# stanfordnlp/mac-network

Measured on NVIDIA H100. Metric: mac_reasoning_steps_per_sec, higher is better.
Workload: dtype bf16

## Files before the change

### mac_network_b200/csrc/read_step.cuh

```cuda
#pragma once
#include "tc_gemm.cuh"

namespace mac {

constexpr int RS_D = 512;
constexpr int RS_BM = 64;
constexpr int RS_KB = RS_D / TC_BK;
constexpr int RS_BLK = RS_BM * TC_BK * 2;
constexpr int RS_A_BYTES = RS_KB * RS_BLK;
constexpr int RS_B_HALF = 256 * TC_BK * 2;
constexpr int RS_W_BYTES = 2 * RS_B_HALF;
constexpr int RS_STAGE = RS_W_BYTES + RS_BLK;
constexpr int RS_STAGES = 2;
constexpr int RS_Q_SLOT = RS_KB;
constexpr int RS_SLOTS = RS_Q_SLOT + 1 + RS_KB;
constexpr int RS_CONSUMERS = 256;
constexpr int RS_THREADS = RS_CONSUMERS + 32;
constexpr int RS_SMEM_BYTES = RS_A_BYTES + RS_STAGES * RS_STAGE + 1024  + 64  +
                              2 * RS_BM * 4  + 2 * RS_D * 4  +
                              2 * RS_D * 4 ;
static_assert(RS_SMEM_BYTES <= 232448, "over the sm_90 per-block shared memory opt-in limit");
static_assert(RS_STAGE % 1024 == 0 && RS_W_BYTES % 1024 == 0, "swizzled operands need 1024-byte alignment");

__device__ __forceinline__ float bf16lo(uint32_t w) { return __uint_as_float(w << 16); }
__device__ __forceinline__ float bf16hi(uint32_t w) { return __uint_as_float(w & 0xffff0000u); }

__device__ __forceinline__ void wgmma_bf16_n256(float (&d)[128], uint64_t adesc, uint64_t bdesc, uint32_t accum) {
  asm volatile(
      "{\n\t.reg .pred p;\n\t"
      "setp.ne.b32 p, %130, 0;\n\t"
      "wgmma.mma_async.sync.aligned.m64n256k16.f32.bf16.bf16 "
      "{%0, %1, %2, %3, %4, %5, %6, %7, %8, %9, %10, %11, %12, %13, %14, %15, %16, %17, %18, %19, %20, %21, %22, %23, %24, %25, %26, %27, %28, %29, %30, %31, %32, %33, %34, %35, %36, %37, %38, %39, %40, %41, %42, %43, %44, %45, %46, %47, %48, %49, %50, %51, %52, %53, %54, %55, %56, %57, %58, %59, %60, %61, %62, %63, %64, %65, %66, %67, %68, %69, %70, %71, %72, %73, %74, %75, %76, %77, %78, %79, %80, %81, %82, %83, %84, %85, %86, %87, %88, %89, %90, %91, %92, %93, %94, %95, %96, %97, %98, %99, %100, %101, %102, %103, %104, %105, %106, %107, %108, %109, %110, %111, %112, %113, %114, %115, %116, %117, %118, %119, %120, %121, %122, %123, %124, %125, %126, %127}, %128, %129, p, 1, 1, 0, 0;\n\t}"
      : "+f"(d[0]), "+f"(d[1]), "+f"(d[2]), "+f"(d[3]), "+f"(d[4]), "+f"(d[5]), "+f"(d[6]), "+f"(d[7]), "+f"(d[8]), "+f"(d[9]), "+f"(d[10]), "+f"(d[11]), "+f"(d[12]), "+f"(d[13]), "+f"(d[14]), "+f"(d[15]), "+f"(d[16]), "+f"(d[17]), "+f"(d[18]), "+f"(d[19]), "+f"(d[20]), "+f"(d[21]), "+f"(d[22]), "+f"(d[23]), "+f"(d[24]), "+f"(d[25]), "+f"(d[26]), "+f"(d[27]), "+f"(d[28]), "+f"(d[29]), "+f"(d[30]), "+f"(d[31]), "+f"(d[32]), "+f"(d[33]), "+f"(d[34]), "+f"(d[35]), "+f"(d[36]), "+f"(d[37]), "+f"(d[38]), "+f"(d[39]), "+f"(d[40]), "+f"(d[41]), "+f"(d[42]), "+f"(d[43]), "+f"(d[44]), "+f"(d[45]), "+f"(d[46]), "+f"(d[47]), "+f"(d[48]), "+f"(d[49]), "+f"(d[50]), "+f"(d[51]), "+f"(d[52]), "+f"(d[53]), "+f"(d[54]), "+f"(d[55]), "+f"(d[56]), "+f"(d[57]), "+f"(d[58]), "+f"(d[59]), "+f"(d[60]), "+f"(d[61]), "+f"(d[62]), "+f"(d[63]), "+f"(d[64]), "+f"(d[65]), "+f"(d[66]), "+f"(d[67]), "+f"(d[68]), "+f"(d[69]), "+f"(d[70]), "+f"(d[71]), "+f"(d[72]), "+f"(d[73]), "+f"(d[74]), "+f"(d[75]), "+f"(d[76]), "+f"(d[77]), "+f"(d[78]), "+f"(d[79]), "+f"(d[80]), "+f"(d[81]), "+f"(d[82]), "+f"(d[83]), "+f"(d[84]), "+f"(d[85]), "+f"(d[86]), "+f"(d[87]), "+f"(d[88]), "+f"(d[89]), "+f"(d[90]), "+f"(d[91]), "+f"(d[92]), "+f"(d[93]), "+f"(d[94]), "+f"(d[95]), "+f"(d[96]), "+f"(d[97]), "+f"(d[98]), "+f"(d[99]), "+f"(d[100]), "+f"(d[101]), "+f"(d[102]), "+f"(d[103]), "+f"(d[104]), "+f"(d[105]), "+f"(d[106]), "+f"(d[107]), "+f"(d[108]), "+f"(d[109]), "+f"(d[110]), "+f"(d[111]), "+f"(d[112]), "+f"(d[113]), "+f"(d[114]), "+f"(d[115]), "+f"(d[116]), "+f"(d[117]), "+f"(d[118]), "+f"(d[119]), "+f"(d[120]), "+f"(d[121]), "+f"(d[122]), "+f"(d[123]), "+f"(d[124]), "+f"(d[125]), "+f"(d[126]), "+f"(d[127])
      : "l"(adesc), "l"(bdesc), "r"(accum));
}
inline bool read_step_supported(int B, int N, int d) {
  return d == RS_D && N >= 1 && N <= 256 && B >= 1 && B < (1 << 22);
}

struct ReadStepParams {
  int M, N;
  const float* y;
  const float* ctrl;
  const float* bm2;
  const float* wr;
  float* logits;
};

__device__ __forceinline__ void rs_consumer_bar() { asm volatile("bar.sync 1, %0;" ::"n"(RS_CONSUMERS) : "memory"); }

__global__ void __launch_bounds__(RS_THREADS, 1)
read_step_kernel(const __grid_constant__ CUtensorMap map_p, const __grid_constant__ CUtensorMap map_q,
                 const __grid_constant__ CUtensorMap map_w1, const __grid_constant__ CUtensorMap map_w2,
                 const ReadStepParams p) {
  extern __shared__ unsigned char smem_dyn[];
  const uint32_t base_u32 = smem_u32(smem_dyn);
  unsigned char* a_tile = smem_dyn + ((1024u - (base_u32 & 1023u)) & 1023u);
  unsigned char* b_ring = a_tile + RS_A_BYTES;
  uint64_t* full = reinterpret_cast<uint64_t*>(b_ring + RS_STAGES * RS_STAGE);
  uint64_t* empty = full + RS_STAGES;
  float* s_lg = reinterpret_cast<float*>(full + 8);
  float* s_ctrl = s_lg + 2 * RS_BM;
  float* s_bm2 = s_ctrl + 2 * RS_D;
  float* s_wr = s_bm2 + RS_D;

  const int warp = threadIdx.x >> 5, lane = threadIdx.x & 31;
  const int row0 = blockIdx.x * RS_BM;
  const int s_lo = row0 / p.N;

  if (threadIdx.x == RS_CONSUMERS) {
    tma_prefetch_desc(&map_p);
    tma_prefetch_desc(&map_q);
    tma_prefetch_desc(&map_w1);
    tma_prefetch_desc(&map_w2);
    for (int i = 0; i < RS_STAGES; ++i) {
      mbar_init(&full[i], 1);
      mbar_init(&empty[i], RS_CONSUMERS / 32);
    }
    fence_mbar_init();
  }
  __syncthreads();

  if (warp == RS_CONSUMERS / 32) {
    if (elect_one()) {
      for (int j = 0; j < RS_SLOTS; ++j) {
        const int s = j % RS_STAGES;
        mbar_wait(&empty[s], ((j / RS_STAGES) & 1) ^ 1);
        unsigned char* dst = b_ring + s * RS_STAGE;
        if (j == RS_Q_SLOT) {
          mbar_expect_tx(&full[s], RS_A_BYTES);
          for (int kb = 0; kb < RS_KB; ++kb) tma_load_2d(dst + kb * RS_BLK, &map_q, kb * TC_BK, row0, &full[s]);
          continue;
        }
        const bool g1 = j < RS_Q_SLOT;
        mbar_expect_tx(&full[s], g1 ? RS_W_BYTES + RS_BLK : RS_W_BYTES);
        const CUtensorMap* m = g1 ? &map_w1 : &map_w2;
        const int k0 = (g1 ? j : j - RS_Q_SLOT - 1) * TC_BK;
        if (g1) tma_load_2d(dst + RS_W_BYTES, &map_p, k0, row0, &full[s]);
        tma_load_2d(dst, m, k0, 0, &full[s]);
        tma_load_2d(dst + RS_B_HALF, m, k0, 256, &full[s]);
      }
    }
    return;
  }

  const int tid = threadIdx.x;
  const int g = warp >> 2;
  const int rl = 16 * (warp & 3) + (lane >> 2);
  const int cq = 256 * g + 2 * (lane & 3);
  const int prow = tid >> 3;
  const int poff = prow * 128 + (tid & 7) * 16;
  const int pcol = ((tid & 7) ^ (prow & 7)) << 3;
  for (int i = tid; i < RS_D; i += RS_CONSUMERS) {
    s_bm2[i] = __ldg(p.bm2 + i);
    s_wr[i] = __ldg(p.wr + i);
  }
  float acc[128];
  const int last_row = min(p.M, row0 + RS_BM) - 1;
  const int nsamp = last_row / p.N - s_lo + 1;
  for (int q = 0; q < min(nsamp, 2); ++q)
    for (int i = tid; i < RS_D; i += RS_CONSUMERS) s_ctrl[q * RS_D + i] = __ldg(p.ctrl + (size_t)(s_lo + q) * RS_D + i);
  int yoff[2];
#pragma unroll
  for (int u = 0; u < 2; ++u) yoff[u] = min(row0 + prow + 32 * u, p.M - 1) / p.N * RS_D + pcol;

  for (int j = 0; j < RS_KB; ++j) {
    const int s = j % RS_STAGES;
    unsigned char* stage = b_ring + s * RS_STAGE;
    float4 y0[2], y1[2];
#pragma unroll
    for (int u = 0; u < 2; ++u) {
      y0[u] = *reinterpret_cast<const float4*>(p.y + yoff[u] + j * TC_BK);
      y1[u] = *reinterpret_cast<const float4*>(p.y + yoff[u] + j * TC_BK + 4);
    }
    mbar_wait(&full[s], (j / RS_STAGES) & 1);
#pragma unroll
    for (int u = 0; u < 2; ++u) {
      uint4* c = reinterpret_cast<uint4*>(stage + RS_W_BYTES + poff + u * 32 * 128);
      const uint4 v = *c;
      *c = make_uint4(pack_bf16(bf16lo(v.x) * y0[u].x, bf16hi(v.x) * y0[u].y), pack_bf16(bf16lo(v.y) * y0[u].z, bf16hi(v.y) * y0[u].w),
                      pack_bf16(bf16lo(v.z) * y1[u].x, bf16hi(v.z) * y1[u].y), pack_bf16(bf16lo(v.w) * y1[u].z, bf16hi(v.w) * y1[u].w));
    }
    fence_proxy_async();
    rs_consumer_bar();
    const uint64_t adesc = make_sw128_kmajor_desc(smem_u32(stage + RS_W_BYTES));
    const uint64_t bdesc = make_sw128_kmajor_desc(smem_u32(stage + g * RS_B_HALF));
    wgmma_fence();
#pragma unroll
    for (int k = 0; k < TC_BK / 16; ++k) wgmma_bf16_n256(acc, adesc + 2 * k, bdesc + 2 * k, (j || k) ? 1u : 0u);
    wgmma_commit();
    wgmma_wait<1>();
    wgmma_hold(acc);
    if (j && lane == 0) mbar_arrive(&empty[(j - 1) % RS_STAGES]);
  }
  wgmma_wait<0>();
  wgmma_hold(acc);
  if (lane == 0) mbar_arrive(&empty[(RS_KB - 1) % RS_STAGES]);

  constexpr int qs = RS_Q_SLOT % RS_STAGES;
  const unsigned char* q_tile = b_ring + qs * RS_STAGE;
  mbar_wait(&full[qs], (RS_Q_SLOT / RS_STAGES) & 1);
#pragma unroll
  for (int h = 0; h < 2; ++h) {
    const int r = rl + 8 * h, row = row0 + r;
#pragma unroll
    for (int j = 0; j < 32; ++j) {
      const int n = cq + 8 * j;
      const int kb = n >> 6, c = (n & 63) >> 3;
      const int off = kb * RS_BLK + r * 128 + ((c ^ (r & 7)) << 4) + (n & 7) * 2;
      const uint32_t q = *reinterpret_cast<const uint32_t*>(q_tile + off);
      const uint32_t hv = row < p.M ? pack_bf16(elu_fast(acc[4 * j + 2 * h] + bf16lo(q)), elu_fast(acc[4 * j + 2 * h + 1] + bf16hi(q)))
                                    : 0u;
      *reinterpret_cast<uint32_t*>(a_tile + off) = hv;
    }
  }
  fence_proxy_async();
  rs_consumer_bar();
  if (lane == 0) mbar_arrive(&empty[qs]);

  const uint32_t a_u = smem_u32(a_tile);
  for (int j = 0; j < RS_KB; ++j) {
    const int jj = RS_Q_SLOT + 1 + j, s = jj % RS_STAGES;
    mbar_wait(&full[s], (jj / RS_STAGES) & 1);
    const uint64_t adesc = make_sw128_kmajor_desc(a_u + j * RS_BLK);
    const uint64_t bdesc = make_sw128_kmajor_desc(smem_u32(b_ring + s * RS_STAGE + g * RS_B_HALF));
    wgmma_fence();
#pragma unroll
    for (int k = 0; k < TC_BK / 16; ++k) wgmma_bf16_n256(acc, adesc + 2 * k, bdesc + 2 * k, (j || k) ? 1u : 0u);
    wgmma_commit();
    wgmma_wait<1>();
    wgmma_hold(acc);
    if (j && lane == 0) mbar_arrive(&empty[(jj - 1) % RS_STAGES]);
  }
  wgmma_wait<0>();
  wgmma_hold(acc);
  if (lane == 0) mbar_arrive(&empty[(RS_SLOTS - 1) % RS_STAGES]);

#pragma unroll
  for (int h = 0; h < 2; ++h) {
    const int r = rl + 8 * h, row = row0 + r;
    const int s = min(row, p.M - 1) / p.N;
    const float* crow = s - s_lo < 2 ? s_ctrl + (s - s_lo) * RS_D : p.ctrl + (size_t)s * RS_D;
    float part = 0.f;
#pragma unroll
    for (int j = 0; j < 32; ++j) {
      const int n = cq + 8 * j;
      const float2 cc = *reinterpret_cast<const float2*>(crow + n);
      const float2 bb = *reinterpret_cast<const float2*>(s_bm2 + n);
      const float2 ww = *reinterpret_cast<const float2*>(s_wr + n);
      const float t0 = elu_fast((acc[4 * j + 2 * h] + bb.x) * cc.x);
      const float t1 = elu_fast((acc[4 * j + 2 * h + 1] + bb.y) * cc.y);
      part = fmaf(t0, ww.x, part);
      part = fmaf(t1, ww.y, part);
    }
    part += __shfl_xor_sync(0xffffffffu, part, 1);
    part += __shfl_xor_sync(0xffffffffu, part, 2);
    if ((lane & 3) == 0) s_lg[g * RS_BM + r] = part;
  }
  rs_consumer_bar();
  if (tid < RS_BM && row0 + tid < p.M) p.logits[row0 + tid] = s_lg[tid] + s_lg[RS_BM + tid];
}

inline int read_step_launch(const void* inv, const void* kb_bf16, const float* y, const float* control,
                            const mac_read_weights* w, float* att, float* info, int B, int N, int d, cudaStream_t stream) {
  if (!read_step_supported(B, N, d)) return MAC_ERR_UNSUPPORTED;
  if (!inv || !kb_bf16 || !y || !control || !w->Wm_bf16 || !w->Wm2_bf16 || !att || !info) return MAC_ERR_INVALID;
  const int M = B * N;
  const TcReadScratch s = tc_read_scratch(const_cast<void*>(inv), B, N, d);
  CUtensorMap mp, mq, mw1, mw2;
  int st = make_tmap_2d(&mp, s.P, 1, (uint64_t)M, (uint64_t)d, (uint64_t)d * 2, RS_BM, TC_BK, 1);
  if (st != MAC_OK) return st;
  st = make_tmap_2d(&mq, s.Q, 1, (uint64_t)M, (uint64_t)d, (uint64_t)d * 2, RS_BM, TC_BK, 1);
  if (st != MAC_OK) return st;
  st = make_tmap_2d(&mw1, w->Wm_bf16, 1, (uint64_t)d, (uint64_t)d, (uint64_t)2 * d * 2, 256, TC_BK, 1);
  if (st != MAC_OK) return st;
  st = make_tmap_2d(&mw2, w->Wm2_bf16, 1, (uint64_t)d, (uint64_t)d, (uint64_t)d * 2, 256, TC_BK, 1);
  if (st != MAC_OK) return st;
  ReadStepParams p{};
  p.M = M; p.N = N; p.y = y; p.ctrl = control; p.bm2 = w->bm2; p.wr = w->wr; p.logits = s.parts;
  MAC_CUDA_TRY(cudaFuncSetAttribute(read_step_kernel, cudaFuncAttributeMaxDynamicSharedMemorySize, RS_SMEM_BYTES));
  read_step_kernel<<<(M + RS_BM - 1) / RS_BM, RS_THREADS, RS_SMEM_BYTES, stream>>>(mp, mq, mw1, mw2, p);
  MAC_LAUNCH_CHECK();
  return mac_kb_attend_fwd(s.parts, 1, w->br, kb_bf16, 1, att, info, B, N, d, stream);
}

}
```

### mac_network_b200/csrc/read_step_fp8.cuh

```cuda
#pragma once
#include <cuda_fp8.h>
#include <cuda_fp16.h>
#include "read_step.cuh"

namespace mac {

constexpr int R8_BK = 128;
constexpr int R8_KB = RS_D / R8_BK;
constexpr int R8_BLK = RS_BM * R8_BK;
constexpr int R8_A_BYTES = R8_KB * R8_BLK;
constexpr int R8_B_HALF = 256 * R8_BK;
constexpr int R8_W_BYTES = 2 * R8_B_HALF;
constexpr int R8_STAGE = R8_W_BYTES + R8_BLK;
constexpr int R8_STAGES = 2;
constexpr int R8_Q_SLOT = R8_KB;
constexpr int R8_SLOTS = R8_Q_SLOT + 1 + R8_KB;
constexpr int R8_SMEM_BYTES = R8_A_BYTES + R8_STAGES * R8_STAGE + 1024  + 64  +
                              2 * RS_BM * 4  + 2 * RS_BM * 4  +
                              2 * RS_D * 4  + 2 * RS_D * 4  +
                              4 * RS_D * 4  + 2 * RS_BM * 4 ;
static_assert(RS_A_BYTES <= R8_STAGE, "the bf16 Q tile must fit in one ring stage");
static_assert(R8_SMEM_BYTES <= 232448, "over the sm_90 per-block shared memory opt-in limit");
static_assert(R8_STAGE % 1024 == 0 && R8_A_BYTES % 1024 == 0, "swizzled operands need 1024-byte alignment");

__device__ __forceinline__ void wgmma_e4m3_n256(float (&d)[128], uint64_t adesc, uint64_t bdesc, uint32_t accum) {
  asm volatile(
      "{\n\t.reg .pred p;\n\t"
      "setp.ne.b32 p, %130, 0;\n\t"
      "wgmma.mma_async.sync.aligned.m64n256k32.f32.e4m3.e4m3 "
      "{%0, %1, %2, %3, %4, %5, %6, %7, %8, %9, %10, %11, %12, %13, %14, %15, %16, %17, %18, %19, %20, %21, %22, %23, %24, %25, %26, %27, %28, %29, %30, %31, %32, %33, %34, %35, %36, %37, %38, %39, %40, %41, %42, %43, %44, %45, %46, %47, %48, %49, %50, %51, %52, %53, %54, %55, %56, %57, %58, %59, %60, %61, %62, %63, %64, %65, %66, %67, %68, %69, %70, %71, %72, %73, %74, %75, %76, %77, %78, %79, %80, %81, %82, %83, %84, %85, %86, %87, %88, %89, %90, %91, %92, %93, %94, %95, %96, %97, %98, %99, %100, %101, %102, %103, %104, %105, %106, %107, %108, %109, %110, %111, %112, %113, %114, %115, %116, %117, %118, %119, %120, %121, %122, %123, %124, %125, %126, %127}, %128, %129, p, 1, 1;\n\t}"
      : "+f"(d[0]), "+f"(d[1]), "+f"(d[2]), "+f"(d[3]), "+f"(d[4]), "+f"(d[5]), "+f"(d[6]), "+f"(d[7]), "+f"(d[8]), "+f"(d[9]), "+f"(d[10]), "+f"(d[11]), "+f"(d[12]), "+f"(d[13]), "+f"(d[14]), "+f"(d[15]), "+f"(d[16]), "+f"(d[17]), "+f"(d[18]), "+f"(d[19]), "+f"(d[20]), "+f"(d[21]), "+f"(d[22]), "+f"(d[23]), "+f"(d[24]), "+f"(d[25]), "+f"(d[26]), "+f"(d[27]), "+f"(d[28]), "+f"(d[29]), "+f"(d[30]), "+f"(d[31]), "+f"(d[32]), "+f"(d[33]), "+f"(d[34]), "+f"(d[35]), "+f"(d[36]), "+f"(d[37]), "+f"(d[38]), "+f"(d[39]), "+f"(d[40]), "+f"(d[41]), "+f"(d[42]), "+f"(d[43]), "+f"(d[44]), "+f"(d[45]), "+f"(d[46]), "+f"(d[47]), "+f"(d[48]), "+f"(d[49]), "+f"(d[50]), "+f"(d[51]), "+f"(d[52]), "+f"(d[53]), "+f"(d[54]), "+f"(d[55]), "+f"(d[56]), "+f"(d[57]), "+f"(d[58]), "+f"(d[59]), "+f"(d[60]), "+f"(d[61]), "+f"(d[62]), "+f"(d[63]), "+f"(d[64]), "+f"(d[65]), "+f"(d[66]), "+f"(d[67]), "+f"(d[68]), "+f"(d[69]), "+f"(d[70]), "+f"(d[71]), "+f"(d[72]), "+f"(d[73]), "+f"(d[74]), "+f"(d[75]), "+f"(d[76]), "+f"(d[77]), "+f"(d[78]), "+f"(d[79]), "+f"(d[80]), "+f"(d[81]), "+f"(d[82]), "+f"(d[83]), "+f"(d[84]), "+f"(d[85]), "+f"(d[86]), "+f"(d[87]), "+f"(d[88]), "+f"(d[89]), "+f"(d[90]), "+f"(d[91]), "+f"(d[92]), "+f"(d[93]), "+f"(d[94]), "+f"(d[95]), "+f"(d[96]), "+f"(d[97]), "+f"(d[98]), "+f"(d[99]), "+f"(d[100]), "+f"(d[101]), "+f"(d[102]), "+f"(d[103]), "+f"(d[104]), "+f"(d[105]), "+f"(d[106]), "+f"(d[107]), "+f"(d[108]), "+f"(d[109]), "+f"(d[110]), "+f"(d[111]), "+f"(d[112]), "+f"(d[113]), "+f"(d[114]), "+f"(d[115]), "+f"(d[116]), "+f"(d[117]), "+f"(d[118]), "+f"(d[119]), "+f"(d[120]), "+f"(d[121]), "+f"(d[122]), "+f"(d[123]), "+f"(d[124]), "+f"(d[125]), "+f"(d[126]), "+f"(d[127])
      : "l"(adesc), "l"(bdesc), "r"(accum));
}

__device__ __forceinline__ float2 e4m3x2_to_float2(uint32_t v) {
  const __half2_raw h = __nv_cvt_fp8x2_to_halfraw2((__nv_fp8x2_storage_t)(v & 0xffffu), __NV_E4M3);
  return __half22float2(*reinterpret_cast<const __half2*>(&h));
}
__device__ __forceinline__ uint32_t float2_to_e4m3x2(float a, float b) {
  return (uint32_t)__nv_cvt_float2_to_fp8x2(make_float2(a, b), __NV_SATFINITE, __NV_E4M3);
}
__device__ __forceinline__ uint32_t scale4_e4m3(uint32_t w, float4 y, float sc) {
  const float2 a = e4m3x2_to_float2(w), b = e4m3x2_to_float2(w >> 16);
  return float2_to_e4m3x2(a.x * (y.x * sc), a.y * (y.y * sc)) | (float2_to_e4m3x2(b.x * (y.z * sc), b.y * (y.w * sc)) << 16);
}

struct ReadStepFp8Params {
  int M, N;
  const float* y;
  const float* ctrl;
  const float* bm2;
  const float* wr;
  const float* sP;
  const float* sw1;
  const float* sw2;
  float* logits;
};

__global__ void __launch_bounds__(RS_THREADS, 1)
read_step_fp8_kernel(const __grid_constant__ CUtensorMap map_p8, const __grid_constant__ CUtensorMap map_q,
                     const __grid_constant__ CUtensorMap map_w1, const __grid_constant__ CUtensorMap map_w2,
                     const ReadStepFp8Params p) {
  extern __shared__ unsigned char smem_dyn[];
  const uint32_t base_u32 = smem_u32(smem_dyn);
  unsigned char* a_tile = smem_dyn + ((1024u - (base_u32 & 1023u)) & 1023u);
  unsigned char* b_ring = a_tile + R8_A_BYTES;
  uint64_t* full = reinterpret_cast<uint64_t*>(b_ring + R8_STAGES * R8_STAGE);
  uint64_t* empty = full + R8_STAGES;
  float* s_lg = reinterpret_cast<float*>(full + 8);
  float* s_hmax = s_lg + 2 * RS_BM;
  float* s_ctrl = s_hmax + 2 * RS_BM;
  float* s_ys = s_ctrl + 2 * RS_D;
  float* s_bm2 = s_ys + 2 * RS_D;
  float* s_wr = s_bm2 + RS_D;
  float* s_sw1 = s_wr + RS_D;
  float* s_sw2 = s_sw1 + RS_D;
  float* s_ay = s_sw2 + RS_D;
  float* s_iay = s_ay + RS_BM;

  const int warp = threadIdx.x >> 5, lane = threadIdx.x & 31;
  const int row0 = blockIdx.x * RS_BM;
  const int s_lo = row0 / p.N;

  if (threadIdx.x == RS_CONSUMERS) {
    tma_prefetch_desc(&map_p8);
    tma_prefetch_desc(&map_q);
    tma_prefetch_desc(&map_w1);
    tma_prefetch_desc(&map_w2);
    for (int i = 0; i < R8_STAGES; ++i) {
      mbar_init(&full[i], 1);
      mbar_init(&empty[i], RS_CONSUMERS / 32);
    }
    fence_mbar_init();
  }
  __syncthreads();

  if (warp == RS_CONSUMERS / 32) {
    if (elect_one()) {
      for (int j = 0; j < R8_SLOTS; ++j) {
        const int s = j % R8_STAGES;
        mbar_wait(&empty[s], ((j / R8_STAGES) & 1) ^ 1);
        unsigned char* dst = b_ring + s * R8_STAGE;
        if (j == R8_Q_SLOT) {
          mbar_expect_tx(&full[s], RS_A_BYTES);
          for (int kb = 0; kb < RS_KB; ++kb) tma_load_2d(dst + kb * RS_BLK, &map_q, kb * TC_BK, row0, &full[s]);
          continue;
        }
        const bool g1 = j < R8_Q_SLOT;
        mbar_expect_tx(&full[s], g1 ? R8_W_BYTES + R8_BLK : R8_W_BYTES);
        const CUtensorMap* m = g1 ? &map_w1 : &map_w2;
        const int k0 = (g1 ? j : j - R8_Q_SLOT - 1) * R8_BK;
        if (g1) tma_load_2d(dst + R8_W_BYTES, &map_p8, k0, row0, &full[s]);
        tma_load_2d(dst, m, k0, 0, &full[s]);
        tma_load_2d(dst + R8_B_HALF, m, k0, 256, &full[s]);
      }
    }
    return;
  }

  const int tid = threadIdx.x;
  const int g = warp >> 2;
  const int rl = 16 * (warp & 3) + (lane >> 2);
  const int cq = 256 * g + 2 * (lane & 3);
  const int prow = tid >> 3;
  const int poff = prow * 128 + (tid & 7) * 16;
  const int pcol = ((tid & 7) ^ (prow & 7)) << 4;
  for (int i = tid; i < RS_D; i += RS_CONSUMERS) {
    s_bm2[i] = __ldg(p.bm2 + i);
    s_wr[i] = __ldg(p.wr + i);
    s_sw1[i] = __ldg(p.sw1 + i);
    s_sw2[i] = __ldg(p.sw2 + i);
  }
  const int last_row = min(p.M, row0 + RS_BM) - 1;
  const int nsamp = last_row / p.N - s_lo + 1;
  for (int q = 0; q < min(nsamp, 2); ++q)
    for (int i = tid; i < RS_D; i += RS_CONSUMERS) s_ctrl[q * RS_D + i] = __ldg(p.ctrl + (size_t)(s_lo + q) * RS_D + i);
  for (int q = warp; q < nsamp; q += RS_CONSUMERS / 32) {
    const float* yr = p.y + (size_t)(s_lo + q) * RS_D;
    float v[RS_D / 32];
    float m = 0.f;
#pragma unroll
    for (int i = 0; i < RS_D / 32; ++i) {
      v[i] = __ldg(yr + lane + 32 * i);
      m = fmaxf(m, fabsf(v[i]));
    }
    m = warp_max(m);
    const float inv = m > 0.f ? 1.f / m : 0.f;
    if (lane == 0) {
      s_ay[q] = m;
      s_iay[q] = inv;
    }
    if (q < 2) {
#pragma unroll
      for (int i = 0; i < RS_D / 32; ++i) s_ys[q * RS_D + lane + 32 * i] = v[i] * inv;
    }
  }
  rs_consumer_bar();
  const float* yrow[2];
  float ysc[2];
#pragma unroll
  for (int u = 0; u < 2; ++u) {
    const int q = min(row0 + prow + 32 * u, p.M - 1) / p.N - s_lo;
    yrow[u] = (q < 2 ? s_ys + q * RS_D : p.y + (size_t)(s_lo + q) * RS_D) + pcol;
    ysc[u] = q < 2 ? 1.f : s_iay[q];
  }

  float acc[128];
  for (int j = 0; j < R8_KB; ++j) {
    const int s = j % R8_STAGES;
    unsigned char* stage = b_ring + s * R8_STAGE;
    mbar_wait(&full[s], (j / R8_STAGES) & 1);
#pragma unroll
    for (int u = 0; u < 2; ++u) {
      uint4* c = reinterpret_cast<uint4*>(stage + R8_W_BYTES + poff + u * 32 * 128);
      const uint4 v = *c;
      const float* yr = yrow[u] + j * R8_BK;
      const float4 y0 = *reinterpret_cast<const float4*>(yr), y1 = *reinterpret_cast<const float4*>(yr + 4);
      const float4 y2 = *reinterpret_cast<const float4*>(yr + 8), y3 = *reinterpret_cast<const float4*>(yr + 12);
      *c = make_uint4(scale4_e4m3(v.x, y0, ysc[u]), scale4_e4m3(v.y, y1, ysc[u]), scale4_e4m3(v.z, y2, ysc[u]),
                      scale4_e4m3(v.w, y3, ysc[u]));
    }
    fence_proxy_async();
    rs_consumer_bar();
    const uint64_t adesc = make_sw128_kmajor_desc(smem_u32(stage + R8_W_BYTES));
    const uint64_t bdesc = make_sw128_kmajor_desc(smem_u32(stage + g * R8_B_HALF));
    wgmma_fence();
#pragma unroll
    for (int k = 0; k < R8_BK / 32; ++k) wgmma_e4m3_n256(acc, adesc + 2 * k, bdesc + 2 * k, (j || k) ? 1u : 0u);
    wgmma_commit();
    wgmma_wait<1>();
    wgmma_hold(acc);
    if (j && lane == 0) mbar_arrive(&empty[(j - 1) % R8_STAGES]);
  }
  wgmma_wait<0>();
  wgmma_hold(acc);
  if (lane == 0) mbar_arrive(&empty[(R8_KB - 1) % R8_STAGES]);

  constexpr int qs = R8_Q_SLOT % R8_STAGES;
  const unsigned char* q_tile = b_ring + qs * R8_STAGE;
  mbar_wait(&full[qs], (R8_Q_SLOT / R8_STAGES) & 1);
#pragma unroll
  for (int h = 0; h < 2; ++h) {
    const int r = rl + 8 * h, row = row0 + r;
    const int rr = min(row, p.M - 1);
    const float rf = __ldg(p.sP + rr) * s_ay[rr / p.N - s_lo];
    float m = 0.f;
#pragma unroll
    for (int j = 0; j < 32; ++j) {
      const int n = cq + 8 * j;
      const int kb = n >> 6, c = (n & 63) >> 3;
      const uint32_t q = *reinterpret_cast<const uint32_t*>(q_tile + kb * RS_BLK + r * 128 + ((c ^ (r & 7)) << 4) + (n & 7) * 2);
      const float2 sw = *reinterpret_cast<const float2*>(s_sw1 + n);
      float h0 = elu_fast(acc[4 * j + 2 * h] * rf * sw.x + bf16lo(q));
      float h1 = elu_fast(acc[4 * j + 2 * h + 1] * rf * sw.y + bf16hi(q));
      if (row >= p.M) h0 = h1 = 0.f;
      acc[4 * j + 2 * h] = h0;
      acc[4 * j + 2 * h + 1] = h1;
      m = fmaxf(m, fmaxf(fabsf(h0), fabsf(h1)));
    }
    m = fmaxf(m, __shfl_xor_sync(0xffffffffu, m, 1));
    m = fmaxf(m, __shfl_xor_sync(0xffffffffu, m, 2));
    if ((lane & 3) == 0) s_hmax[g * RS_BM + r] = m;
  }
  rs_consumer_bar();
  if (lane == 0) mbar_arrive(&empty[qs]);
#pragma unroll
  for (int h = 0; h < 2; ++h) {
    const int r = rl + 8 * h;
    const float am = fmaxf(s_hmax[r], s_hmax[RS_BM + r]);
    const float inv = am > 0.f ? 448.f / am : 0.f;
#pragma unroll
    for (int j = 0; j < 32; ++j) {
      const int n = cq + 8 * j;
      const int kb = n >> 7, c = (n & 127) >> 4;
      *reinterpret_cast<uint16_t*>(a_tile + kb * R8_BLK + r * 128 + ((c ^ (r & 7)) << 4) + (n & 15)) =
          (uint16_t)float2_to_e4m3x2(acc[4 * j + 2 * h] * inv, acc[4 * j + 2 * h + 1] * inv);
    }
  }
  fence_proxy_async();
  rs_consumer_bar();

  const uint32_t a_u = smem_u32(a_tile);
  for (int j = 0; j < R8_KB; ++j) {
    const int jj = R8_Q_SLOT + 1 + j, s = jj % R8_STAGES;
    mbar_wait(&full[s], (jj / R8_STAGES) & 1);
    const uint64_t adesc = make_sw128_kmajor_desc(a_u + j * R8_BLK);
    const uint64_t bdesc = make_sw128_kmajor_desc(smem_u32(b_ring + s * R8_STAGE + g * R8_B_HALF));
    wgmma_fence();
#pragma unroll
    for (int k = 0; k < R8_BK / 32; ++k) wgmma_e4m3_n256(acc, adesc + 2 * k, bdesc + 2 * k, (j || k) ? 1u : 0u);
    wgmma_commit();
    wgmma_wait<1>();
    wgmma_hold(acc);
    if (j && lane == 0) mbar_arrive(&empty[(jj - 1) % R8_STAGES]);
  }
  wgmma_wait<0>();
  wgmma_hold(acc);
  if (lane == 0) mbar_arrive(&empty[(R8_SLOTS - 1) % R8_STAGES]);

#pragma unroll
  for (int h = 0; h < 2; ++h) {
    const int r = rl + 8 * h, row = row0 + r;
    const int s = min(row, p.M - 1) / p.N;
    const float* crow = s - s_lo < 2 ? s_ctrl + (s - s_lo) * RS_D : p.ctrl + (size_t)s * RS_D;
    const float sh = fmaxf(s_hmax[r], s_hmax[RS_BM + r]) / 448.f;
    float part = 0.f;
#pragma unroll
    for (int j = 0; j < 32; ++j) {
      const int n = cq + 8 * j;
      const float2 cc = *reinterpret_cast<const float2*>(crow + n);
      const float2 bb = *reinterpret_cast<const float2*>(s_bm2 + n);
      const float2 ww = *reinterpret_cast<const float2*>(s_wr + n);
      const float2 sw = *reinterpret_cast<const float2*>(s_sw2 + n);
      const float t0 = elu_fast((acc[4 * j + 2 * h] * sh * sw.x + bb.x) * cc.x);
      const float t1 = elu_fast((acc[4 * j + 2 * h + 1] * sh * sw.y + bb.y) * cc.y);
      part = fmaf(t0, ww.x, part);
      part = fmaf(t1, ww.y, part);
    }
    part += __shfl_xor_sync(0xffffffffu, part, 1);
    part += __shfl_xor_sync(0xffffffffu, part, 2);
    if ((lane & 3) == 0) s_lg[g * RS_BM + r] = part;
  }
  rs_consumer_bar();
  if (tid < RS_BM && row0 + tid < p.M) p.logits[row0 + tid] = s_lg[tid] + s_lg[RS_BM + tid];
}

__global__ void pack_weight_fp8_kernel(const float* __restrict__ W, uint8_t* __restrict__ Wt, float* __restrict__ col_scale,
                                       int K, int N) {
  __shared__ float tile[32][33];
  __shared__ float s_max[8][32];
  const int n0 = blockIdx.x * 32, tx = threadIdx.x, ty = threadIdx.y;
  float m = 0.f;
  if (n0 + tx < N)
    for (int k = ty; k < K; k += 8) m = fmaxf(m, fabsf(W[(size_t)k * N + n0 + tx]));
  s_max[ty][tx] = m;
  __syncthreads();
  if (ty == 0) {
    for (int i = 1; i < 8; ++i) m = fmaxf(m, s_max[i][tx]);
    s_max[0][tx] = m;
    if (n0 + tx < N) col_scale[n0 + tx] = m / 448.f;
  }
  __syncthreads();
  for (int k0 = 0; k0 < K; k0 += 32) {
    for (int i = ty; i < 32; i += 8) {
      const int k = k0 + i, n = n0 + tx;
      tile[i][tx] = (k < K && n < N) ? W[(size_t)k * N + n] : 0.f;
    }
    __syncthreads();
    for (int i = ty; i < 32; i += 8) {
      const int n = n0 + i, k = k0 + tx;
      const float am = s_max[0][i];
      if (n < N && k < K)
        Wt[(size_t)n * K + k] = am > 0.f ? __nv_cvt_float_to_fp8(tile[tx][i] / (am / 448.f), __NV_SATFINITE, __NV_E4M3) : 0;
    }
    __syncthreads();
  }
}

__global__ void __launch_bounds__(256) quant_rows_e4m3_kernel(const __nv_bfloat16* __restrict__ P, uint8_t* __restrict__ P8,
                                                             float* __restrict__ sP, int M) {
  const int m = blockIdx.x * 8 + (threadIdx.x >> 5), lane = threadIdx.x & 31;
  if (m >= M) return;
  const uint4* src = reinterpret_cast<const uint4*>(P + (size_t)m * RS_D) + 2 * lane;
  const uint4 a = src[0], b = src[1];
  const uint32_t w[8] = {a.x, a.y, a.z, a.w, b.x, b.y, b.z, b.w};
  float v[16];
  float am = 0.f;
#pragma unroll
  for (int i = 0; i < 8; ++i) {
    v[2 * i] = bf16lo(w[i]);
    v[2 * i + 1] = bf16hi(w[i]);
    am = fmaxf(am, fmaxf(fabsf(v[2 * i]), fabsf(v[2 * i + 1])));
  }
  am = warp_max(am);
  const float s = am / 448.f;
  uint32_t o[4];
#pragma unroll
  for (int i = 0; i < 4; ++i) {
    const uint32_t lo = float2_to_e4m3x2(v[4 * i] / s, v[4 * i + 1] / s);
    const uint32_t hi = float2_to_e4m3x2(v[4 * i + 2] / s, v[4 * i + 3] / s);
    o[i] = am > 0.f ? lo | (hi << 16) : 0u;
  }
  reinterpret_cast<uint4*>(P8 + (size_t)m * RS_D)[lane] = make_uint4(o[0], o[1], o[2], o[3]);
  if (lane == 0) sP[m] = s;
}

struct Fp8ReadScratch {
  uint8_t* P8;
  float* sP;
  __nv_bfloat16* Q;
  float* parts;
  __nv_bfloat16* P;
};
inline size_t fp8_align1k(size_t b) { return (b + 1023) & ~(size_t)1023; }
inline size_t fp8_read_invariant_bytes(int B, int N, int d) {
  const size_t M = (size_t)B * N;
  return fp8_align1k(M * d) + fp8_align1k(M * 4) + 2 * fp8_align1k(M * d * 2) + fp8_align1k(M * 4) + 1024;
}
inline Fp8ReadScratch fp8_read_scratch(void* inv, int B, int N, int d) {
  const size_t M = (size_t)B * N;
  char* o = tc_align1k(inv);
  Fp8ReadScratch s;
  s.P8 = reinterpret_cast<uint8_t*>(o);
  o += fp8_align1k(M * d);
  s.sP = reinterpret_cast<float*>(o);
  o += fp8_align1k(M * 4);
  s.Q = reinterpret_cast<__nv_bfloat16*>(o);
  o += fp8_align1k(M * d * 2);
  s.parts = reinterpret_cast<float*>(o);
  o += fp8_align1k(M * 4);
  s.P = reinterpret_cast<__nv_bfloat16*>(o);
  return s;
}

inline int fp8_read_invariant(const void* kb_bf16, const mac_read_weights* w, void* inv, size_t inv_bytes, int B, int N, int d,
                              cudaStream_t stream) {
  if (!read_step_supported(B, N, d)) return MAC_ERR_UNSUPPORTED;
  if (!kb_bf16 || !w->Wx_bf16 || !w->Wm_bf16) return MAC_ERR_INVALID;
  if (inv_bytes < fp8_read_invariant_bytes(B, N, d)) return MAC_ERR_WORKSPACE;
  const int M = B * N;
  const Fp8ReadScratch s = fp8_read_scratch(inv, B, N, d);
  TcGemmParams p{};
  p.M = M; p.N = d; p.rows_per_batch = N; p.ldo = d;
  p.epi = TC_EPI_ACT; p.act = MAC_ACT_NON; p.bias = w->bx; p.out0 = s.P;
  int st = tc_gemm_launch(kb_bf16, d, nullptr, 0, w->Wx_bf16, p, stream);
  if (st != MAC_OK) return st;
  p.bias = w->bm; p.out0 = s.Q;
  st = tc_gemm_launch(s.P, d, nullptr, 0, reinterpret_cast<const __nv_bfloat16*>(w->Wm_bf16) + d, p, stream, nullptr, 2 * d);
  if (st != MAC_OK) return st;
  quant_rows_e4m3_kernel<<<(M + 7) / 8, 256, 0, stream>>>(s.P, s.P8, s.sP, M);
  MAC_LAUNCH_CHECK();
  return MAC_OK;
}

inline int read_step_fp8_launch(const void* inv, const void* kb_bf16, const float* y, const float* control,
                                const mac_read_weights* w, float* att, float* info, int B, int N, int d, cudaStream_t stream) {
  if (!read_step_supported(B, N, d)) return MAC_ERR_UNSUPPORTED;
  if (!inv || !kb_bf16 || !y || !control || !w->Wm_fp8 || !w->Wm_fp8_scale || !w->Wm2_fp8 || !w->Wm2_fp8_scale || !att || !info)
    return MAC_ERR_INVALID;
  const int M = B * N;
  const Fp8ReadScratch s = fp8_read_scratch(const_cast<void*>(inv), B, N, d);
  CUtensorMap mp, mq, mw1, mw2;
  int st = make_tmap_2d(&mp, s.P8, 2, (uint64_t)M, (uint64_t)d, (uint64_t)d, RS_BM, R8_BK, 1);
  if (st != MAC_OK) return st;
  st = make_tmap_2d(&mq, s.Q, 1, (uint64_t)M, (uint64_t)d, (uint64_t)d * 2, RS_BM, TC_BK, 1);
  if (st != MAC_OK) return st;
  st = make_tmap_2d(&mw1, w->Wm_fp8, 2, (uint64_t)d, (uint64_t)d, (uint64_t)d, 256, R8_BK, 1);
  if (st != MAC_OK) return st;
  st = make_tmap_2d(&mw2, w->Wm2_fp8, 2, (uint64_t)d, (uint64_t)d, (uint64_t)d, 256, R8_BK, 1);
  if (st != MAC_OK) return st;
  ReadStepFp8Params p{};
  p.M = M; p.N = N; p.y = y; p.ctrl = control; p.bm2 = w->bm2; p.wr = w->wr;
  p.sP = s.sP; p.sw1 = w->Wm_fp8_scale; p.sw2 = w->Wm2_fp8_scale; p.logits = s.parts;
  MAC_CUDA_TRY(cudaFuncSetAttribute(read_step_fp8_kernel, cudaFuncAttributeMaxDynamicSharedMemorySize, R8_SMEM_BYTES));
  read_step_fp8_kernel<<<(M + RS_BM - 1) / RS_BM, RS_THREADS, R8_SMEM_BYTES, stream>>>(mp, mq, mw1, mw2, p);
  MAC_LAUNCH_CHECK();
  return mac_kb_attend_fwd(s.parts, 1, w->br, kb_bf16, 1, att, info, B, N, d, stream);
}

}
```

Before: 17800.

## Double read-step row tile so each warpgroup owns 64 rows over split N

The bf16 read-step kernel moves from a 64-row tile, where two warpgroups split the 512 output columns, to a 128-row tile where each warpgroup owns 64 rows and walks the two 256-column halves in sequence. Each ring stage now holds one 256-wide weight half, so every weight byte loaded serves twice as many rows. The Q tile goes straight into the A buffer through its own mbarrier. A four-warp producer warpgroup uses setmaxnreg to hand registers to the consumers. The epilogue writes logits directly, without cross-warpgroup shared reductions, and the fp8 kernel gets its own tile constants so it keeps its old geometry. The cost is twice as many ring slots per tile, half as many CTAs (so less parallelism at small M), and heavier register pressure.

New measurement: 18170 (median of 6 runs). 2.1% higher.

```diff
diff --git a/mac_network_b200/csrc/read_step.cuh b/mac_network_b200/csrc/read_step.cuh
--- a/mac_network_b200/csrc/read_step.cuh
+++ b/mac_network_b200/csrc/read_step.cuh
@@ -4,23 +4,26 @@
 namespace mac {
 
 constexpr int RS_D = 512;
-constexpr int RS_BM = 64;
+constexpr int RS_BM = 128;
+constexpr int RS_WG_BM = 64;
 constexpr int RS_KB = RS_D / TC_BK;
 constexpr int RS_BLK = RS_BM * TC_BK * 2;
+constexpr int RS_WG_BLK = RS_WG_BM * TC_BK * 2;
 constexpr int RS_A_BYTES = RS_KB * RS_BLK;
 constexpr int RS_B_HALF = 256 * TC_BK * 2;
-constexpr int RS_W_BYTES = 2 * RS_B_HALF;
-constexpr int RS_STAGE = RS_W_BYTES + RS_BLK;
+constexpr int RS_STAGE = RS_B_HALF + RS_BLK;
 constexpr int RS_STAGES = 2;
-constexpr int RS_Q_SLOT = RS_KB;
-constexpr int RS_SLOTS = RS_Q_SLOT + 1 + RS_KB;
+constexpr int RS_G2_SLOT = 2 * RS_KB;
+constexpr int RS_SLOTS = 4 * RS_KB;
 constexpr int RS_CONSUMERS = 256;
-constexpr int RS_THREADS = RS_CONSUMERS + 32;
-constexpr int RS_SMEM_BYTES = RS_A_BYTES + RS_STAGES * RS_STAGE + 1024  + 64  +
-                              2 * RS_BM * 4  + 2 * RS_D * 4  +
-                              2 * RS_D * 4 ;
+constexpr int RS_THREADS = RS_CONSUMERS + 128;
+constexpr int RS_PRODUCER_REGS = 40;
+constexpr int RS_CONSUMER_REGS = 232;
+constexpr int RS_SMEM_BYTES = RS_A_BYTES + RS_STAGES * RS_STAGE + 1024  + 64 ;
 static_assert(RS_SMEM_BYTES <= 232448, "over the sm_90 per-block shared memory opt-in limit");
-static_assert(RS_STAGE % 1024 == 0 && RS_W_BYTES % 1024 == 0, "swizzled operands need 1024-byte alignment");
+static_assert(4 * RS_D * 4 <= RS_WG_BLK, "epilogue 2's staged operands fill a warpgroup's rows of a P block");
+static_assert(RS_STAGE % 1024 == 0 && RS_BLK % 1024 == 0 && RS_WG_BLK % 1024 == 0,
+              "swizzled operands need 1024-byte alignment");
 
 __device__ __forceinline__ float bf16lo(uint32_t w) { return __uint_as_float(w << 16); }
 __device__ __forceinline__ float bf16hi(uint32_t w) { return __uint_as_float(w & 0xffff0000u); }
@@ -47,7 +50,10 @@
   float* logits;
 };
 
-__device__ __forceinline__ void rs_consumer_bar() { asm volatile("bar.sync 1, %0;" ::"n"(RS_CONSUMERS) : "memory"); }
+__device__ __forceinline__ void rs_warpgroup_bar(int g) {
+  if (g) asm volatile("bar.sync 2, 128;" ::: "memory");
+  else asm volatile("bar.sync 1, 128;" ::: "memory");
+}
 
 __global__ void __launch_bounds__(RS_THREADS, 1)
 read_step_kernel(const __grid_constant__ CUtensorMap map_p, const __grid_constant__ CUtensorMap map_q,
@@ -59,14 +65,10 @@
   unsigned char* b_ring = a_tile + RS_A_BYTES;
   uint64_t* full = reinterpret_cast<uint64_t*>(b_ring + RS_STAGES * RS_STAGE);
   uint64_t* empty = full + RS_STAGES;
-  float* s_lg = reinterpret_cast<float*>(full + 8);
-  float* s_ctrl = s_lg + 2 * RS_BM;
-  float* s_bm2 = s_ctrl + 2 * RS_D;
-  float* s_wr = s_bm2 + RS_D;
+  uint64_t* q_full = empty + RS_STAGES;
 
   const int warp = threadIdx.x >> 5, lane = threadIdx.x & 31;
   const int row0 = blockIdx.x * RS_BM;
-  const int s_lo = row0 / p.N;
 
   if (threadIdx.x == RS_CONSUMERS) {
     tma_prefetch_desc(&map_p);
@@ -77,148 +79,155 @@
       mbar_init(&full[i], 1);
       mbar_init(&empty[i], RS_CONSUMERS / 32);
     }
+    mbar_init(q_full, 1);
     fence_mbar_init();
   }
   __syncthreads();
 
-  if (warp == RS_CONSUMERS / 32) {
-    if (elect_one()) {
+  if (warp >= RS_CONSUMERS / 32) {
+    asm volatile("setmaxnreg.dec.sync.aligned.u32 %0;" ::"n"(RS_PRODUCER_REGS));
+    if (warp == RS_CONSUMERS / 32 && elect_one()) {
       for (int j = 0; j < RS_SLOTS; ++j) {
         const int s = j % RS_STAGES;
         mbar_wait(&empty[s], ((j / RS_STAGES) & 1) ^ 1);
         unsigned char* dst = b_ring + s * RS_STAGE;
-        if (j == RS_Q_SLOT) {
-          mbar_expect_tx(&full[s], RS_A_BYTES);
-          for (int kb = 0; kb < RS_KB; ++kb) tma_load_2d(dst + kb * RS_BLK, &map_q, kb * TC_BK, row0, &full[s]);
-          continue;
+        const bool g1 = j < RS_G2_SLOT;
+        const int k0 = (j % RS_KB) * TC_BK, n0 = 256 * ((j / RS_KB) & 1);
+        mbar_expect_tx(&full[s], g1 ? RS_STAGE : RS_B_HALF);
+        if (g1) tma_load_2d(dst + RS_B_HALF, &map_p, k0, row0, &full[s]);
+        tma_load_2d(dst, g1 ? &map_w1 : &map_w2, k0, n0, &full[s]);
+        if (j == RS_STAGES - 1) {
+          mbar_expect_tx(q_full, RS_A_BYTES);
+          for (int kb = 0; kb < RS_KB; ++kb) tma_load_2d(a_tile + kb * RS_BLK, &map_q, kb * TC_BK, row0, q_full);
         }
-        const bool g1 = j < RS_Q_SLOT;
-        mbar_expect_tx(&full[s], g1 ? RS_W_BYTES + RS_BLK : RS_W_BYTES);
-        const CUtensorMap* m = g1 ? &map_w1 : &map_w2;
-        const int k0 = (g1 ? j : j - RS_Q_SLOT - 1) * TC_BK;
-        if (g1) tma_load_2d(dst + RS_W_BYTES, &map_p, k0, row0, &full[s]);
-        tma_load_2d(dst, m, k0, 0, &full[s]);
-        tma_load_2d(dst + RS_B_HALF, m, k0, 256, &full[s]);
       }
     }
     return;
   }
 
-  const int tid = threadIdx.x;
+  asm volatile("setmaxnreg.inc.sync.aligned.u32 %0;" ::"n"(RS_CONSUMER_REGS));
   const int g = warp >> 2;
-  const int rl = 16 * (warp & 3) + (lane >> 2);
-  const int cq = 256 * g + 2 * (lane & 3);
-  const int prow = tid >> 3;
-  const int poff = prow * 128 + (tid & 7) * 16;
-  const int pcol = ((tid & 7) ^ (prow & 7)) << 3;
-  for (int i = tid; i < RS_D; i += RS_CONSUMERS) {
-    s_bm2[i] = __ldg(p.bm2 + i);
-    s_wr[i] = __ldg(p.wr + i);
-  }
+  const int t = threadIdx.x & 127;
+  const int rl = RS_WG_BM * g + 16 * (warp & 3) + (lane >> 2);
+  const int cq = 2 * (lane & 3);
+  const int prow = RS_WG_BM * g + (t >> 3);
+  const int poff = prow * 128 + (t & 7) * 16;
+  const int pcol = ((t & 7) ^ (prow & 7)) << 3;
   float acc[128];
-  const int last_row = min(p.M, row0 + RS_BM) - 1;
-  const int nsamp = last_row / p.N - s_lo + 1;
-  for (int q = 0; q < min(nsamp, 2); ++q)
-    for (int i = tid; i < RS_D; i += RS_CONSUMERS) s_ctrl[q * RS_D + i] = __ldg(p.ctrl + (size_t)(s_lo + q) * RS_D + i);
-  int yoff[2];
-#pragma unroll
-  for (int u = 0; u < 2; ++u) yoff[u] = min(row0 + prow + 32 * u, p.M - 1) / p.N * RS_D + pcol;
-
-  for (int j = 0; j < RS_KB; ++j) {
-    const int s = j % RS_STAGES;
-    unsigned char* stage = b_ring + s * RS_STAGE;
-    float4 y0[2], y1[2];
-#pragma unroll
-    for (int u = 0; u < 2; ++u) {
-      y0[u] = *reinterpret_cast<const float4*>(p.y + yoff[u] + j * TC_BK);
-      y1[u] = *reinterpret_cast<const float4*>(p.y + yoff[u] + j * TC_BK + 4);
-    }
-    mbar_wait(&full[s], (j / RS_STAGES) & 1);
-#pragma unroll
-    for (int u = 0; u < 2; ++u) {
-      uint4* c = reinterpret_cast<uint4*>(stage + RS_W_BYTES + poff + u * 32 * 128);
-      const uint4 v = *c;
-      *c = make_uint4(pack_bf16(bf16lo(v.x) * y0[u].x, bf16hi(v.x) * y0[u].y), pack_bf16(bf16lo(v.y) * y0[u].z, bf16hi(v.y) * y0[u].w),
-                      pack_bf16(bf16lo(v.z) * y1[u].x, bf16hi(v.z) * y1[u].y), pack_bf16(bf16lo(v.w) * y1[u].z, bf16hi(v.w) * y1[u].w));
-    }
-    fence_proxy_async();
-    rs_consumer_bar();
-    const uint64_t adesc = make_sw128_kmajor_desc(smem_u32(stage + RS_W_BYTES));
-    const uint64_t bdesc = make_sw128_kmajor_desc(smem_u32(stage + g * RS_B_HALF));
-    wgmma_fence();
-#pragma unroll
-    for (int k = 0; k < TC_BK / 16; ++k) wgmma_bf16_n256(acc, adesc + 2 * k, bdesc + 2 * k, (j || k) ? 1u : 0u);
-    wgmma_commit();
-    wgmma_wait<1>();
+  int yoff[4];
+#pragma unroll
+  for (int u = 0; u < 4; ++u) yoff[u] = min(row0 + prow + 16 * u, p.M - 1) / p.N * RS_D + pcol;
+  const uint32_t a_u = smem_u32(a_tile);
+  float* s_bm2 = reinterpret_cast<float*>(b_ring + RS_B_HALF + g * RS_WG_BLK);
+  float* s_wr = s_bm2 + RS_D;
+  float* s_ctrl = s_wr + RS_D;
+  const int s_lo = min(row0 + RS_WG_BM * g, p.M - 1) / p.N;
+  const int nsamp = (min(p.M, row0 + RS_WG_BM * g + RS_WG_BM) - 1) / p.N - s_lo + 1;
+  float part0[2];
+
+  for (int c = 0; c < 2; ++c) {
+    for (int j = 0; j < RS_KB; ++j) {
+      const int jj = c * RS_KB + j, s = jj % RS_STAGES;
+      unsigned char* stage = b_ring + s * RS_STAGE;
+      float4 y0[4], y1[4];
+#pragma unroll
+      for (int u = 0; u < 4; ++u) {
+        y0[u] = *reinterpret_cast<const float4*>(p.y + yoff[u] + j * TC_BK);
+        y1[u] = *reinterpret_cast<const float4*>(p.y + yoff[u] + j * TC_BK + 4);
+      }
+      mbar_wait(&full[s], (jj / RS_STAGES) & 1);
+#pragma unroll
+      for (int u = 0; u < 4; ++u) {
+        uint4* cp = reinterpret_cast<uint4*>(stage + RS_B_HALF + poff + u * 16 * 128);
+        const uint4 v = *cp;
+        *cp = make_uint4(pack_bf16(bf16lo(v.x) * y0[u].x, bf16hi(v.x) * y0[u].y), pack_bf16(bf16lo(v.y) * y0[u].z, bf16hi(v.y) * y0[u].w),
+                         pack_bf16(bf16lo(v.z) * y1[u].x, bf16hi(v.z) * y1[u].y), pack_bf16(bf16lo(v.w) * y1[u].z, bf16hi(v.w) * y1[u].w));
+      }
+      fence_proxy_async();
+      rs_warpgroup_bar(g);
+      const uint64_t adesc = make_sw128_kmajor_desc(smem_u32(stage + RS_B_HALF + g * RS_WG_BLK));
+      const uint64_t bdesc = make_sw128_kmajor_desc(smem_u32(stage));
+      wgmma_fence();
+#pragma unroll
+      for (int k = 0; k < TC_BK / 16; ++k) wgmma_bf16_n256(acc, adesc + 2 * k, bdesc + 2 * k, (j || k) ? 1u : 0u);
+      wgmma_commit();
+      wgmma_wait<1>();
+      wgmma_hold(acc);
+      if (j && lane == 0) mbar_arrive(&empty[(jj - 1) % RS_STAGES]);
+    }
+    wgmma_wait<0>();
     wgmma_hold(acc);
-    if (j && lane == 0) mbar_arrive(&empty[(j - 1) % RS_STAGES]);
-  }
-  wgmma_wait<0>();
-  wgmma_hold(acc);
-  if (lane == 0) mbar_arrive(&empty[(RS_KB - 1) % RS_STAGES]);
-
-  constexpr int qs = RS_Q_SLOT % RS_STAGES;
-  const unsigned char* q_tile = b_ring + qs * RS_STAGE;
-  mbar_wait(&full[qs], (RS_Q_SLOT / RS_STAGES) & 1);
-#pragma unroll
-  for (int h = 0; h < 2; ++h) {
-    const int r = rl + 8 * h, row = row0 + r;
-#pragma unroll
-    for (int j = 0; j < 32; ++j) {
-      const int n = cq + 8 * j;
-      const int kb = n >> 6, c = (n & 63) >> 3;
-      const int off = kb * RS_BLK + r * 128 + ((c ^ (r & 7)) << 4) + (n & 7) * 2;
-      const uint32_t q = *reinterpret_cast<const uint32_t*>(q_tile + off);
-      const uint32_t hv = row < p.M ? pack_bf16(elu_fast(acc[4 * j + 2 * h] + bf16lo(q)), elu_fast(acc[4 * j + 2 * h + 1] + bf16hi(q)))
-                                    : 0u;
-      *reinterpret_cast<uint32_t*>(a_tile + off) = hv;
+    if (lane == 0) mbar_arrive(&empty[(c * RS_KB + RS_KB - 1) % RS_STAGES]);
+    if (c == 1) {
+      for (int i = t; i < RS_D; i += 128) {
+        s_bm2[i] = __ldg(p.bm2 + i);
+        s_wr[i] = __ldg(p.wr + i);
+      }
+      for (int q = 0; q < min(nsamp, 2); ++q)
+        for (int i = t; i < RS_D; i += 128) s_ctrl[q * RS_D + i] = __ldg(p.ctrl + (size_t)(s_lo + q) * RS_D + i);
+    }
+
+    mbar_wait(q_full, 0);
+#pragma unroll
+    for (int h = 0; h < 2; ++h) {
+      const int r = rl + 8 * h, row = row0 + r;
+#pragma unroll
+      for (int j = 0; j < 32; ++j) {
+        const int n = 256 * c + cq + 8 * j;
+        const int kb = n >> 6, ch = (n & 63) >> 3;
+        uint32_t* hq = reinterpret_cast<uint32_t*>(a_tile + kb * RS_BLK + r * 128 + ((ch ^ (r & 7)) << 4) + (n & 7) * 2);
+        const uint32_t q = *hq;
+        *hq = row < p.M ? pack_bf16(elu_fast(acc[4 * j + 2 * h] + bf16lo(q)), elu_fast(acc[4 * j + 2 * h + 1] + bf16hi(q)))
+                        : 0u;
+      }
     }
   }
   fence_proxy_async();
-  rs_consumer_bar();
-  if (lane == 0) mbar_arrive(&empty[qs]);
-
-  const uint32_t a_u = smem_u32(a_tile);
-  for (int j = 0; j < RS_KB; ++j) {
-    const int jj = RS_Q_SLOT + 1 + j, s = jj % RS_STAGES;
-    mbar_wait(&full[s], (jj / RS_STAGES) & 1);
-    const uint64_t adesc = make_sw128_kmajor_desc(a_u + j * RS_BLK);
-    const uint64_t bdesc = make_sw128_kmajor_desc(smem_u32(b_ring + s * RS_STAGE + g * RS_B_HALF));
-    wgmma_fence();
-#pragma unroll
-    for (int k = 0; k < TC_BK / 16; ++k) wgmma_bf16_n256(acc, adesc + 2 * k, bdesc + 2 * k, (j || k) ? 1u : 0u);
-    wgmma_commit();
-    wgmma_wait<1>();
+  rs_warpgroup_bar(g);
+
+  for (int c = 0; c < 2; ++c) {
+    uint32_t a_c;
+    asm volatile("mov.u32 %0, %1;" : "=r"(a_c) : "r"(a_u));
+    for (int j = 0; j < RS_KB; ++j) {
+      const int jj = RS_G2_SLOT + c * RS_KB + j, s = jj % RS_STAGES;
+      mbar_wait(&full[s], (jj / RS_STAGES) & 1);
+      const uint64_t adesc = make_sw128_kmajor_desc(a_c + j * RS_BLK + g * RS_WG_BLK);
+      const uint64_t bdesc = make_sw128_kmajor_desc(smem_u32(b_ring + s * RS_STAGE));
+      wgmma_fence();
+#pragma unroll
+      for (int k = 0; k < TC_BK / 16; ++k) wgmma_bf16_n256(acc, adesc + 2 * k, bdesc + 2 * k, (j || k) ? 1u : 0u);
+      wgmma_commit();
+      wgmma_wait<1>();
+      wgmma_hold(acc);
+      if (j && lane == 0) mbar_arrive(&empty[(jj - 1) % RS_STAGES]);
+    }
+    wgmma_wait<0>();
     wgmma_hold(acc);
-    if (j && lane == 0) mbar_arrive(&empty[(jj - 1) % RS_STAGES]);
-  }
-  wgmma_wait<0>();
-  wgmma_hold(acc);
-  if (lane == 0) mbar_arrive(&empty[(RS_SLOTS - 1) % RS_STAGES]);
-
-#pragma unroll
-  for (int h = 0; h < 2; ++h) {
-    const int r = rl + 8 * h, row = row0 + r;
-    const int s = min(row, p.M - 1) / p.N;
-    const float* crow = s - s_lo < 2 ? s_ctrl + (s - s_lo) * RS_D : p.ctrl + (size_t)s * RS_D;
-    float part = 0.f;
-#pragma unroll
-    for (int j = 0; j < 32; ++j) {
-      const int n = cq + 8 * j;
-      const float2 cc = *reinterpret_cast<const float2*>(crow + n);
-      const float2 bb = *reinterpret_cast<const float2*>(s_bm2 + n);
-      const float2 ww = *reinterpret_cast<const float2*>(s_wr + n);
-      const float t0 = elu_fast((acc[4 * j + 2 * h] + bb.x) * cc.x);
-      const float t1 = elu_fast((acc[4 * j + 2 * h + 1] + bb.y) * cc.y);
-      part = fmaf(t0, ww.x, part);
-      part = fmaf(t1, ww.y, part);
-    }
-    part += __shfl_xor_sync(0xffffffffu, part, 1);
-    part += __shfl_xor_sync(0xffffffffu, part, 2);
-    if ((lane & 3) == 0) s_lg[g * RS_BM + r] = part;
-  }
-  rs_consumer_bar();
-  if (tid < RS_BM && row0 + tid < p.M) p.logits[row0 + tid] = s_lg[tid] + s_lg[RS_BM + tid];
+    if (lane == 0) mbar_arrive(&empty[(RS_G2_SLOT + c * RS_KB + RS_KB - 1) % RS_STAGES]);
+
+#pragma unroll
+    for (int h = 0; h < 2; ++h) {
+      const int r = rl + 8 * h, row = row0 + r;
+      const int s = min(row, p.M - 1) / p.N;
+      const float* crow = s - s_lo < 2 ? s_ctrl + (s - s_lo) * RS_D : p.ctrl + (size_t)s * RS_D;
+      float part = 0.f;
+#pragma unroll
+      for (int j = 0; j < 32; ++j) {
+        const int n = 256 * c + cq + 8 * j;
+        const float2 cc = *reinterpret_cast<const float2*>(crow + n);
+        const float2 bb = *reinterpret_cast<const float2*>(s_bm2 + n);
+        const float2 ww = *reinterpret_cast<const float2*>(s_wr + n);
+        const float t0 = elu_fast((acc[4 * j + 2 * h] + bb.x) * cc.x);
+        const float t1 = elu_fast((acc[4 * j + 2 * h + 1] + bb.y) * cc.y);
+        part = fmaf(t0, ww.x, part);
+        part = fmaf(t1, ww.y, part);
+      }
+      part += __shfl_xor_sync(0xffffffffu, part, 1);
+      part += __shfl_xor_sync(0xffffffffu, part, 2);
+      if (c == 0) part0[h] = part;
+      else if ((lane & 3) == 0 && row < p.M) p.logits[row] = part0[h] + part;
+    }
+  }
 }
 
 inline int read_step_launch(const void* inv, const void* kb_bf16, const float* y, const float* control,
diff --git a/mac_network_b200/csrc/read_step_fp8.cuh b/mac_network_b200/csrc/read_step_fp8.cuh
--- a/mac_network_b200/csrc/read_step_fp8.cuh
+++ b/mac_network_b200/csrc/read_step_fp8.cuh
@@ -5,9 +5,14 @@
 
 namespace mac {
 
+constexpr int R8_BM = 64;
+constexpr int R8_CONSUMERS = 256;
+constexpr int R8_THREADS = R8_CONSUMERS + 32;
+constexpr int R8_Q_BLK = R8_BM * TC_BK * 2;
+constexpr int R8_Q_BYTES = RS_KB * R8_Q_BLK;
 constexpr int R8_BK = 128;
 constexpr int R8_KB = RS_D / R8_BK;
-constexpr int R8_BLK = RS_BM * R8_BK;
+constexpr int R8_BLK = R8_BM * R8_BK;
 constexpr int R8_A_BYTES = R8_KB * R8_BLK;
 constexpr int R8_B_HALF = 256 * R8_BK;
 constexpr int R8_W_BYTES = 2 * R8_B_HALF;
@@ -16,10 +21,10 @@
 constexpr int R8_Q_SLOT = R8_KB;
 constexpr int R8_SLOTS = R8_Q_SLOT + 1 + R8_KB;
 constexpr int R8_SMEM_BYTES = R8_A_BYTES + R8_STAGES * R8_STAGE + 1024  + 64  +
-                              2 * RS_BM * 4  + 2 * RS_BM * 4  +
+                              2 * R8_BM * 4  + 2 * R8_BM * 4  +
                               2 * RS_D * 4  + 2 * RS_D * 4  +
-                              4 * RS_D * 4  + 2 * RS_BM * 4 ;
-static_assert(RS_A_BYTES <= R8_STAGE, "the bf16 Q tile must fit in one ring stage");
+                              4 * RS_D * 4  + 2 * R8_BM * 4 ;
+static_assert(R8_Q_BYTES <= R8_STAGE, "the bf16 Q tile must fit in one ring stage");
 static_assert(R8_SMEM_BYTES <= 232448, "over the sm_90 per-block shared memory opt-in limit");
 static_assert(R8_STAGE % 1024 == 0 && R8_A_BYTES % 1024 == 0, "swizzled operands need 1024-byte alignment");
 
@@ -57,7 +62,9 @@
   float* logits;
 };
 
-__global__ void __launch_bounds__(RS_THREADS, 1)
+__device__ __forceinline__ void r8_consumer_bar() { asm volatile("bar.sync 1, %0;" ::"n"(R8_CONSUMERS) : "memory"); }
+
+__global__ void __launch_bounds__(R8_THREADS, 1)
 read_step_fp8_kernel(const __grid_constant__ CUtensorMap map_p8, const __grid_constant__ CUtensorMap map_q,
                      const __grid_constant__ CUtensorMap map_w1, const __grid_constant__ CUtensorMap map_w2,
                      const ReadStepFp8Params p) {
@@ -68,42 +75,42 @@
   uint64_t* full = reinterpret_cast<uint64_t*>(b_ring + R8_STAGES * R8_STAGE);
   uint64_t* empty = full + R8_STAGES;
   float* s_lg = reinterpret_cast<float*>(full + 8);
-  float* s_hmax = s_lg + 2 * RS_BM;
-  float* s_ctrl = s_hmax + 2 * RS_BM;
+  float* s_hmax = s_lg + 2 * R8_BM;
+  float* s_ctrl = s_hmax + 2 * R8_BM;
   float* s_ys = s_ctrl + 2 * RS_D;
   float* s_bm2 = s_ys + 2 * RS_D;
   float* s_wr = s_bm2 + RS_D;
   float* s_sw1 = s_wr + RS_D;
   float* s_sw2 = s_sw1 + RS_D;
   float* s_ay = s_sw2 + RS_D;
-  float* s_iay = s_ay + RS_BM;
+  float* s_iay = s_ay + R8_BM;
 
   const int warp = threadIdx.x >> 5, lane = threadIdx.x & 31;
-  const int row0 = blockIdx.x * RS_BM;
+  const int row0 = blockIdx.x * R8_BM;
   const int s_lo = row0 / p.N;
 
-  if (threadIdx.x == RS_CONSUMERS) {
+  if (threadIdx.x == R8_CONSUMERS) {
     tma_prefetch_desc(&map_p8);
     tma_prefetch_desc(&map_q);
     tma_prefetch_desc(&map_w1);
     tma_prefetch_desc(&map_w2);
     for (int i = 0; i < R8_STAGES; ++i) {
       mbar_init(&full[i], 1);
-      mbar_init(&empty[i], RS_CONSUMERS / 32);
+      mbar_init(&empty[i], R8_CONSUMERS / 32);
     }
     fence_mbar_init();
   }
   __syncthreads();
 
-  if (warp == RS_CONSUMERS / 32) {
+  if (warp == R8_CONSUMERS / 32) {
     if (elect_one()) {
       for (int j = 0; j < R8_SLOTS; ++j) {
         const int s = j % R8_STAGES;
         mbar_wait(&empty[s], ((j / R8_STAGES) & 1) ^ 1);
         unsigned char* dst = b_ring + s * R8_STAGE;
         if (j == R8_Q_SLOT) {
-          mbar_expect_tx(&full[s], RS_A_BYTES);
-          for (int kb = 0; kb < RS_KB; ++kb) tma_load_2d(dst + kb * RS_BLK, &map_q, kb * TC_BK, row0, &full[s]);
+          mbar_expect_tx(&full[s], R8_Q_BYTES);
+          for (int kb = 0; kb < RS_KB; ++kb) tma_load_2d(dst + kb * R8_Q_BLK, &map_q, kb * TC_BK, row0, &full[s]);
           continue;
         }
         const bool g1 = j < R8_Q_SLOT;
@@ -125,17 +132,17 @@
   const int prow = tid >> 3;
   const int poff = prow * 128 + (tid & 7) * 16;
   const int pcol = ((tid & 7) ^ (prow & 7)) << 4;
-  for (int i = tid; i < RS_D; i += RS_CONSUMERS) {
+  for (int i = tid; i < RS_D; i += R8_CONSUMERS) {
     s_bm2[i] = __ldg(p.bm2 + i);
     s_wr[i] = __ldg(p.wr + i);
     s_sw1[i] = __ldg(p.sw1 + i);
     s_sw2[i] = __ldg(p.sw2 + i);
   }
-  const int last_row = min(p.M, row0 + RS_BM) - 1;
+  const int last_row = min(p.M, row0 + R8_BM) - 1;
   const int nsamp = last_row / p.N - s_lo + 1;
   for (int q = 0; q < min(nsamp, 2); ++q)
-    for (int i = tid; i < RS_D; i += RS_CONSUMERS) s_ctrl[q * RS_D + i] = __ldg(p.ctrl + (size_t)(s_lo + q) * RS_D + i);
-  for (int q = warp; q < nsamp; q += RS_CONSUMERS / 32) {
+    for (int i = tid; i < RS_D; i += R8_CONSUMERS) s_ctrl[q * RS_D + i] = __ldg(p.ctrl + (size_t)(s_lo + q) * RS_D + i);
+  for (int q = warp; q < nsamp; q += R8_CONSUMERS / 32) {
     const float* yr = p.y + (size_t)(s_lo + q) * RS_D;
     float v[RS_D / 32];
     float m = 0.f;
@@ -155,7 +162,7 @@
       for (int i = 0; i < RS_D / 32; ++i) s_ys[q * RS_D + lane + 32 * i] = v[i] * inv;
     }
   }
-  rs_consumer_bar();
+  r8_consumer_bar();
   const float* yrow[2];
   float ysc[2];
 #pragma unroll
@@ -181,7 +188,7 @@
                       scale4_e4m3(v.w, y3, ysc[u]));
     }
     fence_proxy_async();
-    rs_consumer_bar();
+    r8_consumer_bar();
     const uint64_t adesc = make_sw128_kmajor_desc(smem_u32(stage + R8_W_BYTES));
     const uint64_t bdesc = make_sw128_kmajor_desc(smem_u32(stage + g * R8_B_HALF));
     wgmma_fence();
@@ -209,7 +216,7 @@
     for (int j = 0; j < 32; ++j) {
       const int n = cq + 8 * j;
       const int kb = n >> 6, c = (n & 63) >> 3;
-      const uint32_t q = *reinterpret_cast<const uint32_t*>(q_tile + kb * RS_BLK + r * 128 + ((c ^ (r & 7)) << 4) + (n & 7) * 2);
+      const uint32_t q = *reinterpret_cast<const uint32_t*>(q_tile + kb * R8_Q_BLK + r * 128 + ((c ^ (r & 7)) << 4) + (n & 7) * 2);
       const float2 sw = *reinterpret_cast<const float2*>(s_sw1 + n);
       float h0 = elu_fast(acc[4 * j + 2 * h] * rf * sw.x + bf16lo(q));
       float h1 = elu_fast(acc[4 * j + 2 * h + 1] * rf * sw.y + bf16hi(q));
@@ -220,14 +227,14 @@
     }
     m = fmaxf(m, __shfl_xor_sync(0xffffffffu, m, 1));
     m = fmaxf(m, __shfl_xor_sync(0xffffffffu, m, 2));
-    if ((lane & 3) == 0) s_hmax[g * RS_BM + r] = m;
-  }
-  rs_consumer_bar();
+    if ((lane & 3) == 0) s_hmax[g * R8_BM + r] = m;
+  }
+  r8_consumer_bar();
   if (lane == 0) mbar_arrive(&empty[qs]);
 #pragma unroll
   for (int h = 0; h < 2; ++h) {
     const int r = rl + 8 * h;
-    const float am = fmaxf(s_hmax[r], s_hmax[RS_BM + r]);
+    const float am = fmaxf(s_hmax[r], s_hmax[R8_BM + r]);
     const float inv = am > 0.f ? 448.f / am : 0.f;
 #pragma unroll
     for (int j = 0; j < 32; ++j) {
@@ -238,7 +245,7 @@
     }
   }
   fence_proxy_async();
-  rs_consumer_bar();
+  r8_consumer_bar();
 
   const uint32_t a_u = smem_u32(a_tile);
   for (int j = 0; j < R8_KB; ++j) {
@@ -263,7 +270,7 @@
     const int r = rl + 8 * h, row = row0 + r;
     const int s = min(row, p.M - 1) / p.N;
     const float* crow = s - s_lo < 2 ? s_ctrl + (s - s_lo) * RS_D : p.ctrl + (size_t)s * RS_D;
-    const float sh = fmaxf(s_hmax[r], s_hmax[RS_BM + r]) / 448.f;
+    const float sh = fmaxf(s_hmax[r], s_hmax[R8_BM + r]) / 448.f;
     float part = 0.f;
 #pragma unroll
     for (int j = 0; j < 32; ++j) {
@@ -279,10 +286,10 @@
     }
     part += __shfl_xor_sync(0xffffffffu, part, 1);
     part += __shfl_xor_sync(0xffffffffu, part, 2);
-    if ((lane & 3) == 0) s_lg[g * RS_BM + r] = part;
-  }
-  rs_consumer_bar();
-  if (tid < RS_BM && row0 + tid < p.M) p.logits[row0 + tid] = s_lg[tid] + s_lg[RS_BM + tid];
+    if ((lane & 3) == 0) s_lg[g * R8_BM + r] = part;
+  }
+  r8_consumer_bar();
+  if (tid < R8_BM && row0 + tid < p.M) p.logits[row0 + tid] = s_lg[tid] + s_lg[R8_BM + tid];
 }
 
 __global__ void pack_weight_fp8_kernel(const float* __restrict__ W, uint8_t* __restrict__ Wt, float* __restrict__ col_scale,
@@ -401,9 +408,9 @@
   const int M = B * N;
   const Fp8ReadScratch s = fp8_read_scratch(const_cast<void*>(inv), B, N, d);
   CUtensorMap mp, mq, mw1, mw2;
-  int st = make_tmap_2d(&mp, s.P8, 2, (uint64_t)M, (uint64_t)d, (uint64_t)d, RS_BM, R8_BK, 1);
-  if (st != MAC_OK) return st;
-  st = make_tmap_2d(&mq, s.Q, 1, (uint64_t)M, (uint64_t)d, (uint64_t)d * 2, RS_BM, TC_BK, 1);
+  int st = make_tmap_2d(&mp, s.P8, 2, (uint64_t)M, (uint64_t)d, (uint64_t)d, R8_BM, R8_BK, 1);
+  if (st != MAC_OK) return st;
+  st = make_tmap_2d(&mq, s.Q, 1, (uint64_t)M, (uint64_t)d, (uint64_t)d * 2, R8_BM, TC_BK, 1);
   if (st != MAC_OK) return st;
   st = make_tmap_2d(&mw1, w->Wm_fp8, 2, (uint64_t)d, (uint64_t)d, (uint64_t)d, 256, R8_BK, 1);
   if (st != MAC_OK) return st;
@@ -413,7 +420,7 @@
   p.M = M; p.N = N; p.y = y; p.ctrl = control; p.bm2 = w->bm2; p.wr = w->wr;
   p.sP = s.sP; p.sw1 = w->Wm_fp8_scale; p.sw2 = w->Wm2_fp8_scale; p.logits = s.parts;
   MAC_CUDA_TRY(cudaFuncSetAttribute(read_step_fp8_kernel, cudaFuncAttributeMaxDynamicSharedMemorySize, R8_SMEM_BYTES));
-  read_step_fp8_kernel<<<(M + RS_BM - 1) / RS_BM, RS_THREADS, R8_SMEM_BYTES, stream>>>(mp, mq, mw1, mw2, p);
+  read_step_fp8_kernel<<<(M + R8_BM - 1) / R8_BM, R8_THREADS, R8_SMEM_BYTES, stream>>>(mp, mq, mw1, mw2, p);
   MAC_LAUNCH_CHECK();
   return mac_kb_attend_fwd(s.parts, 1, w->br, kb_bf16, 1, att, info, B, N, d, stream);
 }
diff --git a/profiles/read_step_tiles.py b/profiles/read_step_tiles.py
--- /dev/null
+++ b/profiles/read_step_tiles.py
@@ -0,0 +1,174 @@
+import argparse
+import json
+import os
+import shutil
+import subprocess
+import sys
+import tempfile
+
+ROOT = os.path.dirname(os.path.dirname(os.path.abspath(__file__)))
+LIB_REL = os.path.join("mac_network_b200", "csrc", "libmac_b200.so")
+
+
+def time_read_step(out_npz):
+    import ctypes
+
+    import numpy as np
+    import torch
+    sys.path.insert(0, ROOT)
+    from mac_network_b200 import _lib as L
+    lib = L.load()
+    B, N, d, NR = 64, 196, 512, 6
+    g = torch.Generator(device="cuda").manual_seed(5)
+    W = {k: (torch.randn(*shp, device="cuda", generator=g) * sc).contiguous() for k, shp, sc in (
+        ("Wx", (d, d), d ** -0.5), ("bx", (d,), 0.1), ("Wy", (d, d), d ** -0.5), ("by", (d,), 0.1),
+        ("Wm", (2 * d, d), (2 * d) ** -0.5), ("bm", (d,), 0.1), ("Wm2", (d, d), d ** -0.5), ("bm2", (d,), 0.1),
+        ("wr", (d,), 4 * d ** -0.5))}
+    W16 = []
+    for k in ("Wx", "Wm", "Wm2"):
+        o = torch.empty((W[k].shape[1], W[k].shape[0]), dtype=torch.bfloat16, device="cuda")
+        L.check(lib.mac_pack_weight_bf16(L.ptr(W[k]), L.ptr(o), W[k].shape[0], W[k].shape[1], L.stream_ptr()))
+        W16.append(o)
+    rw = L.ReadWeights(W["Wx"].data_ptr(), W["bx"].data_ptr(), W["Wy"].data_ptr(), W["by"].data_ptr(),
+                       W["Wm"].data_ptr(), W["bm"].data_ptr(), W["Wm2"].data_ptr(), W["bm2"].data_ptr(),
+                       W["wr"].data_ptr(), 0.1, W16[0].data_ptr(), W16[1].data_ptr(), W16[2].data_ptr())
+    nbi = lib.mac_read_invariant_bytes(B, N, d, 1)
+    sets = []
+    for _ in range(NR):
+        kb = torch.nn.functional.elu(torch.randn(B, N, d, device="cuda", generator=g)).to(torch.bfloat16).contiguous()
+        inv = torch.empty(nbi, dtype=torch.uint8, device="cuda")
+        L.check(lib.mac_read_invariant(None, L.ptr(kb), ctypes.byref(rw), 1, L.ptr(inv), nbi, B, N, d, L.stream_ptr()))
+        sets.append((kb, inv, torch.randn(B, d, device="cuda", generator=g), torch.randn(B, d, device="cuda", generator=g),
+                     torch.empty(B, d, device="cuda"), torch.empty(B, N, device="cuda")))
+
+    def run(i):
+        kb, inv, y, c, info, att = sets[i % NR]
+        L.check(lib.mac_read_step_fused(L.ptr(inv), L.ptr(kb), L.ptr(y), L.ptr(c), ctypes.byref(rw), L.ptr(info),
+                                        L.ptr(att), B, N, d, L.stream_ptr()))
+    for i in range(2 * NR):
+        run(i)
+    torch.cuda.synchronize()
+    np.savez(out_npz, info=sets[0][4].cpu().numpy(), att=sets[0][5].cpu().numpy())
+    e0, e1 = torch.cuda.Event(enable_timing=True), torch.cuda.Event(enable_timing=True)
+    iters = 60
+    e0.record()
+    for i in range(iters):
+        run(i)
+    e1.record()
+    torch.cuda.synchronize()
+    print(json.dumps({"us": e0.elapsed_time(e1) * 1e3 / iters}))
+
+
+def l2_read_rate():
+    import torch
+    x = torch.randn(4 * 1024 * 1024, device="cuda")
+    for _ in range(20):
+        x.sum()
+    e0, e1 = torch.cuda.Event(enable_timing=True), torch.cuda.Event(enable_timing=True)
+    iters = 500
+    e0.record()
+    for _ in range(iters):
+        x.sum()
+    e1.record()
+    torch.cuda.synchronize()
+    t = e0.elapsed_time(e1) / 1e3 / iters
+    print(json.dumps({"buffer_bytes": x.numel() * 4, "us_per_read": t * 1e6, "GB_per_s": x.numel() * 4 / t / 1e9}))
+
+
+def child(tree, *args):
+    r = subprocess.run([sys.executable, os.path.join(tree, "profiles", "read_step_tiles.py"), *args], cwd=tree,
+                       capture_output=True, text=True, timeout=1800)
+    if r.returncode:
+        raise RuntimeError("child %s %s failed:\n%s" % (tree, args, r.stderr[-3000:]))
+    return json.loads(r.stdout.strip().splitlines()[-1])
+
+
+def bench(tree, dump=None):
+    cmd = [sys.executable, "bench.py", "--gpus", "1", "--steps", "480", "--warmup", "12"]
+    if dump:
+        cmd += ["--dump-outputs", dump]
+    r = subprocess.run(cmd, cwd=tree, capture_output=True, text=True, timeout=3600)
+    if r.returncode:
+        raise RuntimeError("bench.py in %s failed:\n%s" % (tree, r.stderr[-3000:]))
+    line = [s for s in r.stdout.splitlines() if s.startswith("{")][-1]
+    return json.loads(line)["value"]
+
+
+def same_arrays(a, b):
+    import numpy as np
+    fa, fb = sorted(f for f in os.listdir(a) if f.endswith(".npy")), sorted(f for f in os.listdir(b) if f.endswith(".npy"))
+    if fa != fb or not fa:
+        return {"files": [fa, fb], "identical": False}
+    out = {}
+    for f in fa:
+        x, y = np.load(os.path.join(a, f)), np.load(os.path.join(b, f))
+        out[f] = bool(x.shape == y.shape and x.dtype == y.dtype and x.tobytes() == y.tobytes())
+    return {"per_output": out, "identical": all(out.values())}
+
+
+def main():
+    ap = argparse.ArgumentParser()
+    ap.add_argument("out_dir", nargs="?")
+    ap.add_argument("--parent-lib")
+    ap.add_argument("--rounds", type=int, default=6)
+    ap.add_argument("--bench-runs", type=int, default=3)
+    ap.add_argument("--parts", default="kernel,bench,l2")
+    ap.add_argument("--time-read-step", metavar="NPZ", help=argparse.SUPPRESS)
+    ap.add_argument("--l2-read", action="store_true", help=argparse.SUPPRESS)
+    a = ap.parse_args()
+    if a.time_read_step:
+        return time_read_step(a.time_read_step)
+    if a.l2_read:
+        return l2_read_rate()
+    import numpy as np
+    os.makedirs(a.out_dir, exist_ok=True)
+    q = subprocess.run(["nvidia-smi", "--query-gpu=name,power.limit,clocks.max.sm", "--format=csv,noheader"],
+                       capture_output=True, text=True, timeout=60)
+    name, power, clock = [s.strip() for s in q.stdout.strip().splitlines()[0].split(",")]
+    path = os.path.join(a.out_dir, "read_step_tiles_h100.json")
+    res = json.load(open(path)) if os.path.exists(path) else {}
+    res["device"] = {"name": name, "power_limit": power, "max_sm_clock": clock}
+    parts = a.parts.split(",")
+    with tempfile.TemporaryDirectory() as tmp:
+        parent = os.path.join(tmp, "parent")
+        skip_files = shutil.ignore_patterns(".git", "__pycache__", "*.ncu-rep", "*.o")
+        out_abs = os.path.abspath(a.out_dir)
+
+        def skip(d, names):
+            return set(skip_files(d, names)) | {n for n in names if os.path.abspath(os.path.join(d, n)) == out_abs}
+        shutil.copytree(ROOT, parent, ignore=skip)
+        shutil.copy(a.parent_lib, os.path.join(parent, LIB_REL))
+        trees = {"parent": parent, "new": ROOT}
+
+        def spread(xs):
+            return {"median": float(np.median(xs)), "min": float(min(xs)), "max": float(max(xs)),
+                    "runs": [round(float(x), 4) for x in xs]}
+        if "kernel" in parts:
+            us = {k: [] for k in trees}
+            for r in range(a.rounds):
+                for k in (("parent", "new") if r % 2 == 0 else ("new", "parent")):
+                    us[k].append(child(trees[k], "--time-read-step", os.path.join(tmp, k + ".npz"))["us"])
+                    print("read step", k, us[k][-1], flush=True)
+            o = {k: np.load(os.path.join(tmp, k + ".npz")) for k in trees}
+            res["read_step_fused_us"] = {k: spread(v) for k, v in us.items()}
+            res["read_step_fused_us"]["outputs_bit_identical"] = all(
+                o["parent"][f].tobytes() == o["new"][f].tobytes() for f in ("info", "att"))
+        if "bench" in parts:
+            vals = {k: [] for k in trees}
+            for r in range(a.bench_runs):
+                for k in (("parent", "new") if r % 2 == 0 else ("new", "parent")):
+                    vals[k].append(bench(trees[k], os.path.join(tmp, "dump_" + k) if r == 0 else None))
+                    print("headline", k, vals[k][-1], flush=True)
+            res["headline_reasoning_steps_per_s"] = {k: spread(v) for k, v in vals.items()}
+            res["headline_reasoning_steps_per_s"]["ratio_of_medians"] = float(np.median(vals["new"]) /
+                                                                              np.median(vals["parent"]))
+            res["bench_dump_outputs"] = same_arrays(os.path.join(tmp, "dump_parent"), os.path.join(tmp, "dump_new"))
+        if "l2" in parts:
+            res["l2_resident_read"] = child(ROOT, "--l2-read")
+    with open(path, "w") as f:
+        json.dump(res, f, indent=1)
+    print(json.dumps(res))
+
+
+if __name__ == "__main__":
+    main()
```
